# MAC-VO/MAC-VO

Measured on AMD Instinct MI355X. Metric: stereo frames/sec at 640x480 (hot path: cost volume + lookup, keypoint selection, covariance, PGO), higher is better.
Workload: dtype f32 via f16x2 (volume: fp32 operands row-scaled by powers of two and split into two fp16 pieces, three products, fp32 accumulate, scales undone exactly) + f32 (lookup/covariance) + f64 (PGO)

## Files before the change

mac-vo_amd/csrc/common.h:

```cpp
#pragma once
#include <hip/hip_runtime.h>
#include <stdint.h>
#include "macvo_hip.h"

#define MV_WAVE 64

#ifndef MV_PLAIN_STORES
#define MV_VOL_STORE(v, p) __builtin_nontemporal_store((v), (p))
#define MV_VOL_STORE_ASM_MOD " nt"
#else
#define MV_VOL_STORE(v, p) (*(p) = (v))
#define MV_VOL_STORE_ASM_MOD ""
#endif

struct mvEpiArgs {
    const float* flow;
    const float* logcov;
    int cov_is_log;
    float bl_fx, bl_fx_sq;
    float *disparity, *disparity_cov, *depth, *depth_cov, *match_flow, *match_cov;
    uint8_t* bad_mask;
};
#ifdef __HIPCC__
__device__ __forceinline__ void mv_epilogue_pixel(const mvEpiArgs& a, int plane, int i) {
    const float fx0 = a.flow[i];
    const float lc0 = a.logcov[i];
    const float dcov = a.cov_is_log ? expf(lc0 * 2.f) : lc0;
    const float d = fabsf(fx0);
    if (a.disparity) a.disparity[i] = d;
    if (a.disparity_cov) a.disparity_cov[i] = dcov;
    if (a.depth) a.depth[i] = a.bl_fx * (1.f / d);
    if (a.depth_cov) {
        const float d2 = d * d;
        const float err2 = dcov * (1.f / d2);
        a.depth_cov[i] = a.bl_fx_sq * (err2 / d2);
    }
    if (a.bad_mask) a.bad_mask[i] = fx0 <= 0.f;
    if (a.match_flow) {
        a.match_flow[i] = a.flow[2 * plane + i];
        a.match_flow[plane + i] = a.flow[3 * plane + i];
    }
    if (a.match_cov) {
        const float l0 = a.logcov[2 * plane + i], l1 = a.logcov[3 * plane + i];
        a.match_cov[i] = a.cov_is_log ? expf(l0 * 2.f) : l0;
        a.match_cov[plane + i] = a.cov_is_log ? expf(l1 * 2.f) : l1;
        a.match_cov[2 * plane + i] = 0.f;
    }
}
template <bool D, bool M>
__device__ __forceinline__ void mv_epilogue_pixel_partial(const mvEpiArgs& a, int plane, int i) {
    const float fx0 = a.flow[i];
    const float d = fabsf(fx0);
    if (a.disparity) a.disparity[i] = d;
    if (a.depth) a.depth[i] = a.bl_fx * (1.f / d);
    if constexpr (D) {
        const float lc0 = a.logcov[i];
        const float dcov = a.cov_is_log ? expf(lc0 * 2.f) : lc0;
        if (a.disparity_cov) a.disparity_cov[i] = dcov;
        if (a.depth_cov) {
            const float d2 = d * d;
            const float err2 = dcov * (1.f / d2);
            a.depth_cov[i] = a.bl_fx_sq * (err2 / d2);
        }
    }
    if (a.bad_mask) a.bad_mask[i] = fx0 <= 0.f;
    if (a.match_flow) {
        a.match_flow[i] = a.flow[2 * plane + i];
        a.match_flow[plane + i] = a.flow[3 * plane + i];
    }
    if constexpr (M) {
        if (a.match_cov) {
            const float l0 = a.logcov[2 * plane + i], l1 = a.logcov[3 * plane + i];
            a.match_cov[i] = a.cov_is_log ? expf(l0 * 2.f) : l0;
            a.match_cov[plane + i] = a.cov_is_log ? expf(l1 * 2.f) : l1;
            a.match_cov[2 * plane + i] = 0.f;
        }
    }
}
#endif

struct mvLaneCounts {
    int32_t n[MV_MAX_LANES];
};

#define MV_CHECK_ARG(cond) \
    do {                   \
        if (!(cond)) return MV_ERR_INVALID_ARG; \
    } while (0)

#ifndef MV_NO_SMALL_PRIO
#define MV_SMALL_KERNEL_PRIO() __builtin_amdgcn_s_setprio(3)
#else
#define MV_SMALL_KERNEL_PRIO() ((void)0)
#endif

#ifdef MV_PRIO_CHAIN
#define MV_CHAIN_KERNEL_PRIO() __builtin_amdgcn_s_setprio(3)
#else
#define MV_CHAIN_KERNEL_PRIO() ((void)0)
#endif

static inline int mv_launch_status() {
    return hipGetLastError() == hipSuccess ? MV_OK : MV_ERR_LAUNCH;
}

static inline int mv_ceil_div(int a, int b) { return (a + b - 1) / b; }

static inline bool mv_cov_modifiers_ok(int32_t m) {
    bool ended = false;
    for (int s = 0; s < 8; ++s) {
        const int k = (int)(((uint32_t)m >> (4 * s)) & 15u);
        if (k == 0) { ended = true; continue; }
        if (ended || s >= 4 || (k != MV_COVMOD_DIAG && k != MV_COVMOD_NORMALIZE)) return false;
    }
    return true;
}

#include "backend_desc.h"

__device__ __forceinline__ float wave_sum(float v) {
#pragma unroll
    for (int o = 32; o > 0; o >>= 1) v += __shfl_xor(v, o, 64);
    return v;
}
__device__ __forceinline__ double wave_sum(double v) {
#pragma unroll
// ... 9 lines not shown
```

mac-vo_amd/csrc/corr_lookup.hip:

```cpp
#include "common.h"

namespace {

struct AxisEntry { float w; int c; };

template <int K, int QPW, int STRIDE, int CELLS>
__device__ __forceinline__ void tap_pairs(const float* blk, const AxisEntry (*ax)[2 * K], int lane, float (&res)[(QPW * K * K + 63) / 64]) {
    constexpr int KK = K * K, NPAIR = QPW * KK, NR = (NPAIR + 63) / 64;
#pragma unroll
    for (int r = 0; r < NR; ++r) {
        const int pair = min(r * 64 + lane, NPAIR - 1);
        const int s = pair / KK, tap = pair - s * KK;
        const int ti = tap / K, tj = tap - ti * K;
        const AxisEntry X = ax[s][ti], Y = ax[s][K + tj];
        const float w = X.w, n = Y.w;
        const bool inblk = ((X.c & Y.c) & 256) != 0;
        const float* p = &blk[s * CELLS + (Y.c & 255) * STRIDE + (X.c & 255)];
        const float e = 1.f - w, so = 1.f - n;
        const float vnw = inblk ? p[0] : 0.f, vne = inblk ? p[1] : 0.f;
        const float vsw = inblk ? p[STRIDE] : 0.f, vse = inblk ? p[STRIDE + 1] : 0.f;
        float r0 = vnw * (so * e);
        r0 = r0 + vne * (so * w);
        r0 = r0 + vsw * (n * e);
        r0 = r0 + vse * (n * w);
        res[r] = r0;
    }
}

template <int K, int QPW, int QPB>
__device__ __forceinline__ void tap_pairs_out(float (*outs)[QPB + 1], int wave, int lane, const float (&res)[(QPW * K * K + 63) / 64]) {
    constexpr int KK = K * K, NPAIR = QPW * KK, NR = (NPAIR + 63) / 64;
#pragma unroll
    for (int r = 0; r < NR; ++r) {
        const int pair = r * 64 + lane;
        if (pair < NPAIR) {
            const int s = pair / KK, tap = pair - s * KK;
            outs[tap][wave * QPW + s] = res[r];
        }
    }
}

template <int R, int QPW, int QPB, typename VT = float>
__global__ __launch_bounds__(64 * (QPB / QPW)) void corr_lookup_kernel(const VT* __restrict__ vol,
                                                                        const float* __restrict__ coords,
                                                                        float* __restrict__ out, int N1, int H2, int W2) {
    constexpr int K = 2 * R + 1;
    constexpr int KK = K * K;
    constexpr int BS = K + 3;
    constexpr int CELLS = BS * BS;
    constexpr int NWAVE = QPB / QPW;
    constexpr int NTHR = 64 * NWAVE;
    constexpr int RPR = 64 / BS;
    constexpr int LPR = RPR * BS;
    constexpr int NROUND = (BS + RPR - 1) / RPR;
    constexpr bool TRIM = (BS - 2) % RPR == 0;
    constexpr int NINNER = (BS - 2) / RPR;
    constexpr int QPA = 64 / (2 * K);
    constexpr int APASS = (QPW + QPA - 1) / QPA;
    static_assert(QPW <= 32 && (QPW & (QPW - 1)) == 0 && QPB % QPW == 0, "bad lookup tiling");

    constexpr int BLK_STRIDE = QPW * CELLS;
    constexpr int BLK_FLOATS = NWAVE * BLK_STRIDE;
    constexpr int OUT_FLOATS = KK * (QPB + 1);
    __shared__ float smem[BLK_FLOATS > OUT_FLOATS ? BLK_FLOATS : OUT_FLOATS];
    float* blk = smem + (threadIdx.x >> 6) * BLK_STRIDE;
    float (*outs)[QPB + 1] = reinterpret_cast<float (*)[QPB + 1]>(smem);

    MV_SMALL_KERNEL_PRIO();
    const int b = blockIdx.y;
    const int q0 = blockIdx.x * QPB;
    const int t = threadIdx.x, lane = t & 63, wave = t >> 6;
    const int slice = H2 * W2;

    const int qmine = q0 + wave * QPW + (lane & (QPW - 1));
    float x = 0.f, y = 0.f;
    if (qmine < N1) {
        x = coords[((size_t)b * 2 + 0) * N1 + qmine];
        y = coords[((size_t)b * 2 + 1) * N1 + qmine];
    }
    const float xc = fminf(fmaxf(x, -1.0e6f), 1.0e6f), yc = fminf(fmaxf(y, -1.0e6f), 1.0e6f);
    const int bx = ((xc == xc) ? (int)floorf(xc) : 0) - R - 1;
    const int by = ((yc == yc) ? (int)floorf(yc) : 0) - R - 1;
    const float frx = xc - floorf(xc), fry = yc - floorf(yc);
    const int margin = ((frx < 0.01f) ? 1 : 0) | ((frx > 0.99f) ? 2 : 0) | ((fry < 0.01f) ? 4 : 0) | ((fry > 0.99f) ? 8 : 0);

    const int cyl = lane / BS, cxl = lane - cyl * BS;
    float v[QPW][NROUND];
#pragma unroll
    for (int s = 0; s < QPW; ++s) {
        const int sbx = __builtin_amdgcn_readlane(bx, s), sby = __builtin_amdgcn_readlane(by, s);
        const int q = q0 + wave * QPW + s;
        const VT* __restrict__ base = vol + ((size_t)b * N1 + q) * slice;
        const int gx = sbx + cxl;
        if (TRIM) {
            const int mg = __builtin_amdgcn_readlane(margin, s);
            const bool okx = lane < LPR && q < N1 && gx >= 0 && gx < W2 && (cxl != 0 || (mg & 1)) && (cxl != BS - 1 || (mg & 2));
#pragma unroll
            for (int k = 0; k < NINNER; ++k) {
                const int row = 1 + k * RPR + cyl, gy = sby + row;
                const bool ok = okx && gy >= 0 && gy < H2;
                v[s][k] = ok ? (float)base[gy * W2 + gx] : 0.f;
            }
            v[s][NROUND - 1] = 0.f;
            if (mg & 12) {
                const int row = cyl == 0 ? 0 : BS - 1, gy = sby + row;
                const bool ok = okx && cyl < 2 && ((mg >> (cyl == 0 ? 2 : 3)) & 1) && gy >= 0 && gy < H2;
                v[s][NROUND - 1] = ok ? (float)base[gy * W2 + gx] : 0.f;
            }
        } else {
            const bool okx = lane < LPR && q < N1 && gx >= 0 && gx < W2;
#pragma unroll
            for (int k = 0; k < NROUND; ++k) {
                const int row = k * RPR + cyl, gy = sby + row;
                const bool ok = okx && row < BS && gy >= 0 && gy < H2;
                v[s][k] = ok ? (float)base[gy * W2 + gx] : 0.f;
            }
        }
    }

    const float wm1 = (float)(W2 - 1), hm1 = (float)(H2 - 1);
    const int asq = lane / (2 * K), aa = lane - asq * (2 * K);
    const bool a_is_y = aa >= K;
    const int aoff = (a_is_y ? aa - K : aa) - R;
    const float adim = a_is_y ? hm1 : wm1;
    __shared__ AxisEntry ax_all[NWAVE][QPW][2 * K];
    AxisEntry (*ax)[2 * K] = ax_all[wave];
#pragma unroll
    for (int ps = 0; ps < APASS; ++ps) {
        const int s = ps * QPA + asq;
        const float qx = __shfl(x, s, 64), qy = __shfl(y, s, 64);
        const int obx = __shfl(bx, s, 64), oby = __shfl(by, s, 64);
        const float cs = (a_is_y ? qy : qx) + (float)aoff;
        const float g = (2.f * cs) / adim - 1.f;
        const float ic = (g + 1.f) * (adim / 2.f);
        const float f0 = floorf(ic);
        const int c = (int)fminf(fmaxf(f0, -2.0e6f), 2.0e6f) - (a_is_y ? oby : obx);
        const bool inb = c >= 0 && c <= BS - 2;
        if (asq < QPA && s < QPW) ax[s][aa] = AxisEntry{ic - f0, min(max(c, 0), BS - 2) | (inb ? 256 : 0)};
    }

#pragma unroll
    for (int s = 0; s < QPW; ++s) {
        if (TRIM) {
#pragma unroll
            for (int k = 0; k < NINNER; ++k)
                if (lane < LPR) blk[s * CELLS + BS + k * LPR + lane] = v[s][k];
            if (lane < 2 * BS) blk[s * CELLS + (lane < BS ? lane : (BS - 2) * BS + lane)] = v[s][NROUND - 1];
        } else {
#pragma unroll
            for (int k = 0; k < NROUND; ++k)
                if (lane < LPR && k * LPR + lane < CELLS) blk[s * CELLS + k * LPR + lane] = v[s][k];
        }
    }
    __syncthreads();

    float res[(QPW * KK + 63) / 64];
    tap_pairs<K, QPW, BS, CELLS>(blk, ax, lane, res);
    __syncthreads();
    tap_pairs_out<K, QPW, QPB>(outs, wave, lane, res);
    __syncthreads();

    for (int idx = t; idx < KK * QPB; idx += NTHR) {
        const int k = idx / QPB, c = idx - k * QPB;
        if (q0 + c < N1) out[((size_t)b * KK + k) * N1 + q0 + c] = outs[k][c];
    }
}


template <int QPW, int QPB, typename VT = float>
__global__ __launch_bounds__(64 * (QPB / QPW)) void corr_lookup_tiled_kernel(const VT* __restrict__ vol,
                                                                              const float* __restrict__ coords,
                                                                              float* __restrict__ out, int N1, int H2, int W2) {
    constexpr int R = 4, K = 9, KK = 81;
    constexpr int BS = 16;
    constexpr int BSP = 18, CELLS = BS * BSP;
    constexpr int NWAVE = QPB / QPW, NTHR = 64 * NWAVE;
    constexpr int QPA = 64 / (2 * K);
    constexpr int APASS = (QPW + QPA - 1) / QPA;
    constexpr int BLK_STRIDE = QPW * CELLS;
    constexpr int BLK_FLOATS = NWAVE * BLK_STRIDE;
    constexpr int OUT_FLOATS = KK * (QPB + 1);
    __shared__ float smem[BLK_FLOATS > OUT_FLOATS ? BLK_FLOATS : OUT_FLOATS];
    float* blk = smem + (threadIdx.x >> 6) * BLK_STRIDE;
    float (*outs)[QPB + 1] = reinterpret_cast<float (*)[QPB + 1]>(smem);

    MV_SMALL_KERNEL_PRIO();
    const int b = blockIdx.y;
    const int q0 = blockIdx.x * QPB;
    const int t = threadIdx.x, lane = t & 63, wave = t >> 6;
    const int tpr = W2 >> 2, tpc = (H2 + 3) >> 2, slice = tpc * tpr * 16;

    const int qmine = q0 + wave * QPW + (lane & (QPW - 1));
    float x = 0.f, y = 0.f;
    if (qmine < N1) {
        x = coords[((size_t)b * 2 + 0) * N1 + qmine];
        y = coords[((size_t)b * 2 + 1) * N1 + qmine];
    }
    const float xc = fminf(fmaxf(x, -1.0e6f), 1.0e6f), yc = fminf(fmaxf(y, -1.0e6f), 1.0e6f);
    const int bx = ((xc == xc) ? (int)floorf(xc) : 0) - R - 1;
    const int by = ((yc == yc) ? (int)floorf(yc) : 0) - R - 1;
    const float frx = xc - floorf(xc), fry = yc - floorf(yc);
    const int x_lo = bx + ((frx < 0.01f) ? 0 : 1), x_hi = bx + ((frx > 0.99f) ? K + 2 : K + 1);
    const int y_lo = by + ((fry < 0.01f) ? 0 : 1), y_hi = by + ((fry > 0.99f) ? K + 2 : K + 1);
    const int tox = bx >> 2, toy = by >> 2;

    constexpr bool H16 = sizeof(VT) == 2;
    constexpr int NLD = H16 ? 2 : 4;
    const int ti = H16 ? (lane >> 3) & 3 : lane >> 4, cell = H16 ? (lane & 7) * 2 : lane & 15;
    const int half_row = H16 ? lane >> 5 : 0;
    float v[QPW][4];
#pragma unroll
    for (int s = 0; s < QPW; ++s) {
        const int stx = __builtin_amdgcn_readlane(tox, s), sty = __builtin_amdgcn_readlane(toy, s);
        const int sxl = __builtin_amdgcn_readlane(x_lo, s), sxh = __builtin_amdgcn_readlane(x_hi, s);
        const int syl = __builtin_amdgcn_readlane(y_lo, s), syh = __builtin_amdgcn_readlane(y_hi, s);
        const int q = q0 + wave * QPW + s;
        const VT* __restrict__ base = vol + ((size_t)b * N1 + q) * slice;
        const int tx = stx + ti;
        const bool okx = q < N1 && tx >= 0 && tx < tpr && 4 * tx + 3 >= sxl && 4 * tx <= sxh;
#pragma unroll
        for (int k = 0; k < NLD; ++k) {
            const int ty = sty + (H16 ? 2 * k + half_row : k);
            const bool ok = okx && ty >= 0 && ty < tpc && 4 * ty + 3 >= syl && 4 * ty <= syh;
            if constexpr (H16) {
                union { uint32_t u; _Float16 h[2]; } two;
                two.u = ok ? *reinterpret_cast<const uint32_t*>(base + ((ty * tpr + tx) << 4) + cell) : 0u;
                v[s][2 * k] = (float)two.h[0];
                v[s][2 * k + 1] = (float)two.h[1];
            } else {
                v[s][k] = ok ? (float)base[((ty * tpr + tx) << 4) + cell] : 0.f;
            }
        }
    }

    const float wm1 = (float)(W2 - 1), hm1 = (float)(H2 - 1);
    const int asq = lane / (2 * K), aa = lane - asq * (2 * K);
    const bool a_is_y = aa >= K;
    const int aoff = (a_is_y ? aa - K : aa) - R;
    const float adim = a_is_y ? hm1 : wm1;
    __shared__ AxisEntry ax_all[NWAVE][QPW][2 * K];
    AxisEntry (*ax)[2 * K] = ax_all[wave];
#pragma unroll
    for (int ps = 0; ps < APASS; ++ps) {
        const int s = ps * QPA + asq;
        const float qx = __shfl(x, s, 64), qy = __shfl(y, s, 64);
        const int obx = __shfl(tox, s, 64) * 4, oby = __shfl(toy, s, 64) * 4;
        const float cs = (a_is_y ? qy : qx) + (float)aoff;
        const float g = (2.f * cs) / adim - 1.f;
        const float ic = (g + 1.f) * (adim / 2.f);
        const float f0 = floorf(ic);
        const int c = (int)fminf(fmaxf(f0, -2.0e6f), 2.0e6f) - (a_is_y ? oby : obx);
        const bool inb = c >= 0 && c <= BS - 2;
        if (asq < QPA && s < QPW) ax[s][aa] = AxisEntry{ic - f0, min(max(c, 0), BS - 2) | (inb ? 256 : 0)};
    }

#pragma unroll
    for (int s = 0; s < QPW; ++s)
#pragma unroll
        for (int k = 0; k < NLD; ++k) {
            if constexpr (H16)
                *reinterpret_cast<float2*>(&blk[s * CELLS + (4 * (2 * k + half_row) + (cell >> 2)) * BSP + 4 * ti + (cell & 3)]) =
                    make_float2(v[s][2 * k], v[s][2 * k + 1]);
            else
                blk[s * CELLS + (4 * k + (cell >> 2)) * BSP + 4 * ti + (cell & 3)] = v[s][k];
        }
    __syncthreads();

    float res[(QPW * KK + 63) / 64];
    tap_pairs<K, QPW, BSP, CELLS>(blk, ax, lane, res);
    __syncthreads();
    tap_pairs_out<K, QPW, QPB>(outs, wave, lane, res);
    __syncthreads();
    for (int idx = t; idx < KK * QPB; idx += NTHR) {
        const int k = idx / QPB, c = idx - k * QPB;
        if (q0 + c < N1) out[((size_t)b * KK + k) * N1 + q0 + c] = outs[k][c];
    }
}

}

#include <stdlib.h>
static int lookup_small_threshold() {
    static int v = -1;
    if (v < 0) {
        const char* e = getenv("MV_LOOKUP_SMALL");
        v = e ? atoi(e) : 65536;
    }
    return v;
}

extern "C" int mv_corr_lookup(const float* vol, const float* coords, float* out, int B, int H1, int W1,
                              int H2, int W2, int radius, mvStream_t stream) {
    MV_CHECK_ARG(vol && coords && out);
    MV_CHECK_ARG(B > 0 && H1 > 0 && W1 > 0 && H2 > 1 && W2 > 1);
    if (radius < 1 || radius > 4) return MV_ERR_UNSUPPORTED;
    if (B > 65535) return MV_ERR_UNSUPPORTED;
    const int N1 = H1 * W1;
    hipStream_t s = (hipStream_t)stream;
    const bool small = (size_t)B * N1 <= (size_t)lookup_small_threshold();
    static int small_qpb = -1;
    if (small_qpb < 0) { const char* e = getenv("MV_LOOKUP_QPB"); small_qpb = (e && atoi(e) == 8) ? 8 : 16; }
#define MV_LOOKUP(R)                                                                                                  \
    if (small && small_qpb == 8)                                                                                      \
        hipLaunchKernelGGL((corr_lookup_kernel<R, 2, 8>), dim3(mv_ceil_div(N1, 8), B), dim3(256), 0, s, vol, coords,  \
                           out, N1, H2, W2);                                                                          \
    else if (small)                                                                                                   \
        hipLaunchKernelGGL((corr_lookup_kernel<R, 2, 16>), dim3(mv_ceil_div(N1, 16), B), dim3(512), 0, s, vol, coords, \
                           out, N1, H2, W2);                                                                          \
    else                                                                                                              \
        hipLaunchKernelGGL((corr_lookup_kernel<R, 4, 32>), dim3(mv_ceil_div(N1, 32), B), dim3(512), 0, s, vol, coords, \
                           out, N1, H2, W2)
    switch (radius) {
        case 1: MV_LOOKUP(1); break;
        case 2: MV_LOOKUP(2); break;
        case 3: MV_LOOKUP(3); break;
        default: MV_LOOKUP(4); break;
    }
#undef MV_LOOKUP
    return mv_launch_status();
}

extern "C" int mv_corr_lookup_vol16(const void* vol, const float* coords, float* out, int B, int H1, int W1, int H2, int W2, int radius,
                                    mvStream_t stream) {
    MV_CHECK_ARG(vol && coords && out);
    MV_CHECK_ARG(B > 0 && H1 > 0 && W1 > 0 && H2 > 1 && W2 > 1);
    if (radius != 4 || B > 65535) return MV_ERR_UNSUPPORTED;
    const int N1 = H1 * W1;
    hipStream_t s = (hipStream_t)stream;
    const _Float16* v = reinterpret_cast<const _Float16*>(vol);
    if ((size_t)B * N1 <= (size_t)lookup_small_threshold())
        hipLaunchKernelGGL((corr_lookup_kernel<4, 2, 16, _Float16>), dim3(mv_ceil_div(N1, 16), B), dim3(512), 0, s, v, coords, out, N1, H2, W2);
    else
        hipLaunchKernelGGL((corr_lookup_kernel<4, 4, 32, _Float16>), dim3(mv_ceil_div(N1, 32), B), dim3(512), 0, s, v, coords, out, N1, H2, W2);
    return mv_launch_status();
}

extern "C" int mv_corr_lookup_tiled(const float* vol, const float* coords, float* out, int B, int H1, int W1, int H2, int W2,
                                    int radius, mvStream_t stream) {
    MV_CHECK_ARG(vol && coords && out);
    MV_CHECK_ARG(B > 0 && H1 > 0 && W1 > 0 && H2 > 1 && W2 > 1);
    if (radius != 4 || (H2 % 4) || (W2 % 4) || B > 65535) return MV_ERR_UNSUPPORTED;
    const int N1 = H1 * W1;
    hipStream_t s = (hipStream_t)stream;
    if ((size_t)B * N1 <= (size_t)lookup_small_threshold())
        hipLaunchKernelGGL((corr_lookup_tiled_kernel<2, 16>), dim3(mv_ceil_div(N1, 16), B), dim3(512), 0, s, vol, coords, out, N1, H2, W2);
    else
        hipLaunchKernelGGL((corr_lookup_tiled_kernel<4, 32>), dim3(mv_ceil_div(N1, 32), B), dim3(512), 0, s, vol, coords, out, N1, H2, W2);
    return mv_launch_status();
}


extern "C" int mv_corr_lookup_tiled_vol16(const void* vol, const float* coords, float* out, int B, int H1, int W1, int H2, int W2, int radius,
                                          mvStream_t stream) {
    MV_CHECK_ARG(vol && coords && out);
    MV_CHECK_ARG(B > 0 && H1 > 0 && W1 > 0 && H2 > 1 && W2 > 1);
    MV_CHECK_ARG(((uintptr_t)vol & 31) == 0);
    if (radius != 4 || (W2 % 4) || B > 65535) return MV_ERR_UNSUPPORTED;
    const int N1 = H1 * W1;
    hipStream_t s = (hipStream_t)stream;
// ... 38 lines not shown
```

mac-vo_amd/csrc/kp_select.hip:

```cpp
#include "common.h"
#include <math.h>

namespace {

#ifdef MV_KP_PROFILE
__device__ long long g_kp_stamps[16];
#define KP_STAMP(i) do { if (threadIdx.x == 0) g_kp_stamps[i] = wall_clock64(); } while (0)
#else
#define KP_STAMP(i)
#endif

constexpr int TILE_W = 64;
constexpr int TILE_H = 16;
constexpr int MAX_R = 7;
constexpr unsigned CAND_FLAG = 0x80000000u;

struct KpWs {
    unsigned long long* cand_bits;
    unsigned* rec_idx;
    float* rec_q;
    float* rec_d;
    int* counters;
    size_t lane_bytes;

    __device__ __forceinline__ KpWs lane(int l) const {
        const size_t o = (size_t)l * lane_bytes;
        return KpWs{(unsigned long long*)((char*)cand_bits + o), (unsigned*)((char*)rec_idx + o), (float*)((char*)rec_q + o),
                    (float*)((char*)rec_d + o), (int*)((char*)counters + o), lane_bytes};
    }
};

__device__ __forceinline__ float flow_quality(const float* __restrict__ fc, int plane, int idx) {
    const float c0 = fc[idx], c1 = fc[plane + idx], c2 = fc[2 * plane + idx];
    return (c0 + c1) - 2.f * c2;
}

__device__ __forceinline__ float nanmin(float a, float b) { return (a < b || a != a) ? a : b; }

template <bool FUSE>
__global__ __launch_bounds__(256) void kp_nms_kernel(const float* __restrict__ fc, const float* __restrict__ d0,
                                                      const float* __restrict__ d0c, const float* __restrict__ d1,
                                                      const float* __restrict__ d1c,
                                                      const uint8_t* __restrict__ mask_a,
                                                      const uint8_t* __restrict__ mask_b, mvKpSelectParams p,
                                                      KpWs ws_all, int words_per_row, mvEpiArgs ef) {
    MV_CHAIN_KERNEL_PRIO();
    const KpWs ws = ws_all.lane(blockIdx.z);
    {
        const size_t lp = (size_t)blockIdx.z * p.H * p.W;
        if (fc) fc += 3 * lp;
        if (d0) d0 += lp;
        if (d0c) d0c += lp;
        if (d1) d1 += lp;
        if (d1c) d1c += lp;
        if (mask_a) mask_a += lp;
        if (mask_b) mask_b += lp;
        if (FUSE) {
            ef.flow += 4 * lp; ef.logcov += 4 * lp;
            if (ef.disparity) ef.disparity += lp;
            if (ef.disparity_cov) ef.disparity_cov += lp;
            if (ef.depth) ef.depth += lp;
            if (ef.depth_cov) ef.depth_cov += lp;
            if (ef.bad_mask) ef.bad_mask += lp;
            if (ef.match_flow) ef.match_flow += 2 * lp;
            if (ef.match_cov) ef.match_cov += 3 * lp;
        }
    }
    __shared__ float tile[TILE_H + 2 * MAX_R][TILE_W + 2 * MAX_R + 1];
    __shared__ float hmin[TILE_H + 2 * MAX_R][TILE_W + 1];
    __shared__ int wg_count, wg_base;
    const int H = p.H, W = p.W, plane = H * W;
    const int r = p.kernel_size >> 1;
    const int x0 = blockIdx.x * TILE_W, y0 = blockIdx.y * TILE_H;
    const int tx = threadIdx.x, ty = threadIdx.y;
    const int tid = ty * 64 + tx;
    const bool mapping = p.mode == MV_KP_MAPPING;
    if (tid == 0) wg_count = 0;

    if (!mapping) {
        const int tw = TILE_W + 2 * r, th = TILE_H + 2 * r;
        constexpr int NST = ((TILE_W + 2 * MAX_R) * (TILE_H + 2 * MAX_R) + 255) / 256;
        float qv[NST];
#pragma unroll
        for (int i = 0; i < NST; ++i) {
            const int e = i * 256 + tid;
            const int ly = e / tw, lx = e - ly * tw;
            const int gx = x0 + lx - r, gy = y0 + ly - r;
            float q = INFINITY;
            if (e < tw * th && gx >= 0 && gx < W && gy >= 0 && gy < H) {
                const int idx = gy * W + gx;
                if (FUSE) {
                    const float l0 = ef.logcov[2 * plane + idx], l1 = ef.logcov[3 * plane + idx];
                    const float c0 = ef.cov_is_log ? expf(l0 * 2.f) : l0, c1 = ef.cov_is_log ? expf(l1 * 2.f) : l1;
                    q = (c0 + c1) - 2.f * 0.f;
                } else if (p.mode == MV_KP_NODEPTH) {
                    q = flow_quality(fc, plane, idx);
                } else {
                    q = d0c[idx] + d1c[idx];
                    if (fc) q = q * flow_quality(fc, plane, idx);
                }
            }
            qv[i] = q;
        }
#pragma unroll
        for (int i = 0; i < NST; ++i) {
            const int e = i * 256 + tid;
            const int ly = e / tw, lx = e - ly * tw;
            if (e < tw * th) tile[ly][lx] = qv[i];
        }
        __syncthreads();
        for (int e = tid; e < th * TILE_W; e += 256) {
            const int ly = e >> 6, lx = e & 63;
            float m = tile[ly][lx];
            for (int dx = 1; dx <= 2 * r; ++dx) m = nanmin(m, tile[ly][lx + dx]);
            hmin[ly][lx] = m;
        }
    }
    __syncthreads();

    bool nms_px[TILE_H / 4];
    bool cand_px[TILE_H / 4];
    float q_px[TILE_H / 4];
    int my_nms = 0;
#pragma unroll
    for (int it = 0; it < TILE_H / 4; ++it) {
        const int ly = ty * (TILE_H / 4) + it;
        const int gx = x0 + tx, gy = y0 + ly;
        const bool inimg = gx < W && gy < H;
        const int idx = gy * W + gx;
        bool nms = false, cand = false;
        float q = 0.f;
        if (FUSE && inimg) mv_epilogue_pixel(ef, plane, idx);
        if (inimg) {
            const bool border = p.mask_width > 0 && gx >= p.mask_width && gx < W - p.mask_width &&
                                gy >= p.mask_width && gy < H - p.mask_width;
            if (mapping) {
                cand = border && (d0[idx] < p.max_depth) && (d0c[idx] < p.max_depth_cov);
            } else {
                q = tile[ly + r][tx + r];
                float m = hmin[ly][tx];
                for (int dy = 1; dy <= 2 * r; ++dy) m = nanmin(m, hmin[ly + dy][tx]);
                nms = (q == m);
                cand = nms && border;
                if (cand && p.mode == MV_KP_FULL) cand = (d0[idx] < p.max_depth) && (d1[idx] < p.max_depth);
            }
            if (cand && mask_a) cand = mask_a[idx] != 0;
            if (cand && mask_b) cand = mask_b[idx] != 0;
        }
        const unsigned long long cand_word = __ballot(cand);
        if (tx == 0 && gy < H) ws.cand_bits[(size_t)gy * words_per_row + blockIdx.x] = cand_word;
        nms_px[it] = nms;
        cand_px[it] = cand;
        q_px[it] = q;
        my_nms += nms;
    }
    if (mapping) return;

    int my_off = 0;
    if (my_nms) my_off = atomicAdd(&wg_count, my_nms);
    __syncthreads();
#ifdef MV_KP_FAKE_ATOMIC
    if (tid == 0) wg_base = (blockIdx.y * gridDim.x + blockIdx.x) * 16;
#else
    if (tid == 0) wg_base = wg_count ? atomicAdd(&ws.counters[0], wg_count) : 0;
#endif
    __syncthreads();
    int pos = wg_base + my_off;
#pragma unroll
    for (int it = 0; it < TILE_H / 4; ++it) {
        if (nms_px[it]) {
            const int gx = x0 + tx, gy = y0 + ty * (TILE_H / 4) + it;
            const int idx = gy * W + gx;
            ws.rec_idx[pos] = (unsigned)(((gy * words_per_row + blockIdx.x) << 6) | tx) | (cand_px[it] ? CAND_FLAG : 0u);
            if (p.mode == MV_KP_NODEPTH) {
                ws.rec_q[pos] = q_px[it];
            } else {
                ws.rec_q[pos] = fc ? flow_quality(fc, plane, idx) : 0.f;
                ws.rec_d[pos] = d0c[idx];
            }
            ++pos;
        }
    }
}

__device__ __forceinline__ unsigned float_key(float f) {
    if (f != f) return 0xFFFFFFFFu;
    const unsigned u = __float_as_uint(f);
    return (u & 0x80000000u) ? ~u : (u | 0x80000000u);
}
__device__ __forceinline__ float key_float(unsigned k) {
    const unsigned u = (k & 0x80000000u) ? (k & 0x7FFFFFFFu) : ~k;
    return __uint_as_float(u);
}

#ifndef MV_KP_FINISH_THREADS
#define MV_KP_FINISH_THREADS 1024
#endif

constexpr int RANK_CAP = 256;
constexpr unsigned NAN_KEY = 0xFFFFFFFFu;

template <int NT>
__device__ __forceinline__ int block_exclusive_scan(int v, int* wave_tot , int& total) {
    constexpr int NW = NT / 64;
    const int tid = threadIdx.x;
    int incl = v;
#pragma unroll
    for (int o = 1; o < 64; o <<= 1) {
        const int t = __shfl_up(incl, o, 64);
        if ((tid & 63) >= o) incl += t;
    }
    __syncthreads();
    if ((tid & 63) == 63) wave_tot[tid >> 6] = incl;
    __syncthreads();
    int off = 0;
    total = 0;
#pragma unroll
    for (int w = 0; w < NW; ++w) {
        const int t = wave_tot[w];
        if (w < (tid >> 6)) off += t;
        total += t;
    }
    return off + incl - v;
}

template <int NT, bool CACHED, int RPT, typename F>
__device__ __forceinline__ void for_each_key(const float* __restrict__ vals, int n, const unsigned (&keys)[RPT], F&& f) {
    const int tid = threadIdx.x;
    if (CACHED) {
        const int nr = (n + NT - 1) / NT;
#pragma unroll
        for (int r = 0; r < RPT; ++r)
            if (r < nr && r * NT + tid < n) f(keys[r]);
    } else {
        for (int i = tid; i < n; i += NT) f(float_key(vals[i]));
    }
}

struct MedianLds {
    unsigned hist[2048];
    unsigned lst[RANK_CAP];
    unsigned red_lo[16], red_hi[16];
    int red_cnt[16];
    int wave_tot[16];
    int sh[4];
    unsigned res;
};

template <int NT, bool CACHED, int RPT>
__device__ float block_nanmedian(const float* __restrict__ vals, int n, const unsigned (&keys)[RPT], MedianLds& L) {
    constexpr int NW = NT / 64, BPT = 2048 / NT;
    const int tid = threadIdx.x;
    unsigned lo = NAN_KEY, hi = 0u;
    int cnt = 0;
    for_each_key<NT, CACHED, RPT>(vals, n, keys, [&](unsigned k) {
        if (k != NAN_KEY) {
            lo = min(lo, k);
            hi = max(hi, k);
            ++cnt;
        }
    });
#pragma unroll
    for (int o = 32; o > 0; o >>= 1) {
        lo = min(lo, (unsigned)__shfl_xor((int)lo, o, 64));
// ... 459 lines not shown
```

Measured before the change: 7092.

## Reuse staged LDS blocks for lookup outputs and restructure NMS record compaction

The correlation lookup kernel now writes tap results back into each wave's own staged block region, using only a wave-level LDS handover instead of two block-wide barriers and a separate output array. It redistributes taps across lanes with padded strides to cut LDS bank conflicts, and remaps output channels. The keypoint NMS kernel replaces the shared atomic counter with per-wave ballot counts and mbcnt-based positions. It also issues the fused epilogue loads early and overlaps the epilogue stores with the global atomic. This adds complex lane-mapping logic that is specialised for K=9, which raises the risk of indexing mistakes.

```diff
diff --git a/mac-vo_amd/csrc/common.h b/mac-vo_amd/csrc/common.h
--- a/mac-vo_amd/csrc/common.h
+++ b/mac-vo_amd/csrc/common.h
@@ -42,6 +42,35 @@
     }
     if (a.match_cov) {
         const float l0 = a.logcov[2 * plane + i], l1 = a.logcov[3 * plane + i];
+        a.match_cov[i] = a.cov_is_log ? expf(l0 * 2.f) : l0;
+        a.match_cov[plane + i] = a.cov_is_log ? expf(l1 * 2.f) : l1;
+        a.match_cov[2 * plane + i] = 0.f;
+    }
+}
+struct mvEpiPixel { float fx0, lc0, f2, f3, l0, l1; };
+__device__ __forceinline__ mvEpiPixel mv_epilogue_load(const mvEpiArgs& a, int plane, int i) {
+    return mvEpiPixel{a.flow[i], a.logcov[i], a.flow[2 * plane + i], a.flow[3 * plane + i], a.logcov[2 * plane + i], a.logcov[3 * plane + i]};
+}
+__device__ __forceinline__ void mv_epilogue_store(const mvEpiArgs& a, int plane, int i, const mvEpiPixel& v) {
+    const float fx0 = v.fx0;
+    const float lc0 = v.lc0;
+    const float dcov = a.cov_is_log ? expf(lc0 * 2.f) : lc0;
+    const float d = fabsf(fx0);
+    if (a.disparity) a.disparity[i] = d;
+    if (a.disparity_cov) a.disparity_cov[i] = dcov;
+    if (a.depth) a.depth[i] = a.bl_fx * (1.f / d);
+    if (a.depth_cov) {
+        const float d2 = d * d;
+        const float err2 = dcov * (1.f / d2);
+        a.depth_cov[i] = a.bl_fx_sq * (err2 / d2);
+    }
+    if (a.bad_mask) a.bad_mask[i] = fx0 <= 0.f;
+    if (a.match_flow) {
+        a.match_flow[i] = v.f2;
+        a.match_flow[plane + i] = v.f3;
+    }
+    if (a.match_cov) {
+        const float l0 = v.l0, l1 = v.l1;
         a.match_cov[i] = a.cov_is_log ? expf(l0 * 2.f) : l0;
         a.match_cov[plane + i] = a.cov_is_log ? expf(l1 * 2.f) : l1;
         a.match_cov[2 * plane + i] = 0.f;
diff --git a/mac-vo_amd/csrc/corr_lookup.hip b/mac-vo_amd/csrc/corr_lookup.hip
--- a/mac-vo_amd/csrc/corr_lookup.hip
+++ b/mac-vo_amd/csrc/corr_lookup.hip
@@ -2,41 +2,98 @@
 
 namespace {
 
-struct AxisEntry { float w; int c; };
+struct alignas(8) AxisEntry { float w; int c; };
+
+__device__ __forceinline__ void wave_lds_handover() {
+    __builtin_amdgcn_fence(__ATOMIC_RELEASE, "wavefront");
+    __builtin_amdgcn_wave_barrier();
+    __builtin_amdgcn_fence(__ATOMIC_ACQUIRE, "wavefront");
+}
+
+template <int K, int STRIDE>
+__device__ __forceinline__ float tap_one(const float* qblk, const AxisEntry* qax, int ti, int tj) {
+    const AxisEntry X = qax[ti], Y = qax[K + tj];
+    const float w = X.w, n = Y.w;
+    const bool inblk = ((X.c & Y.c) & 256) != 0;
+    const float* p = &qblk[(Y.c & 255) * STRIDE + (X.c & 255)];
+    const float e = 1.f - w, so = 1.f - n;
+    const float vnw = inblk ? p[0] : 0.f, vne = inblk ? p[1] : 0.f;
+    const float vsw = inblk ? p[STRIDE] : 0.f, vse = inblk ? p[STRIDE + 1] : 0.f;
+    float r0 = vnw * (so * e);
+    r0 = r0 + vne * (so * w);
+    r0 = r0 + vsw * (n * e);
+    r0 = r0 + vse * (n * w);
+    return r0;
+}
+
+template <int K, int QPW>
+constexpr int strip_pitch() { return K * K + ((K == 9 && QPW == 4) ? 2 : 1); }
+template <int K, int QPW, int CELLS>
+constexpr int wave_floats() { return QPW * CELLS + ((K == 9 && QPW == 4) ? 12 : 0); }
+
+template <int K>
+__device__ __forceinline__ int tap_channel(int u) {
+    if constexpr (K == 9) return u < 72 ? u + (u >> 3) : 9 * (u - 72) + 8;
+    else return u;
+}
 
 template <int K, int QPW, int STRIDE, int CELLS>
-__device__ __forceinline__ void tap_pairs(const float* blk, const AxisEntry (*ax)[2 * K], int lane, float (&res)[(QPW * K * K + 63) / 64]) {
-    constexpr int KK = K * K, NPAIR = QPW * KK, NR = (NPAIR + 63) / 64;
-#pragma unroll
-    for (int r = 0; r < NR; ++r) {
-        const int pair = min(r * 64 + lane, NPAIR - 1);
-        const int s = pair / KK, tap = pair - s * KK;
-        const int ti = tap / K, tj = tap - ti * K;
-        const AxisEntry X = ax[s][ti], Y = ax[s][K + tj];
-        const float w = X.w, n = Y.w;
-        const bool inblk = ((X.c & Y.c) & 256) != 0;
-        const float* p = &blk[s * CELLS + (Y.c & 255) * STRIDE + (X.c & 255)];
-        const float e = 1.f - w, so = 1.f - n;
-        const float vnw = inblk ? p[0] : 0.f, vne = inblk ? p[1] : 0.f;
-        const float vsw = inblk ? p[STRIDE] : 0.f, vse = inblk ? p[STRIDE + 1] : 0.f;
-        float r0 = vnw * (so * e);
-        r0 = r0 + vne * (so * w);
-        r0 = r0 + vsw * (n * e);
-        r0 = r0 + vse * (n * w);
-        res[r] = r0;
-    }
-}
-
-template <int K, int QPW, int QPB>
-__device__ __forceinline__ void tap_pairs_out(float (*outs)[QPB + 1], int wave, int lane, const float (&res)[(QPW * K * K + 63) / 64]) {
-    constexpr int KK = K * K, NPAIR = QPW * KK, NR = (NPAIR + 63) / 64;
-#pragma unroll
-    for (int r = 0; r < NR; ++r) {
-        const int pair = r * 64 + lane;
-        if (pair < NPAIR) {
-            const int s = pair / KK, tap = pair - s * KK;
-            outs[tap][wave * QPW + s] = res[r];
+__device__ __forceinline__ void tap_phase(float* blk, const AxisEntry (*ax)[2 * K], int lane) {
+    constexpr int KK = K * K, P = strip_pitch<K, QPW>();
+    static_assert(P <= CELLS, "the output strip must fit in the wave's staged blocks");
+    if constexpr (K == 9) {
+        static_assert(QPW % 2 == 0, "the leftover rounds pair queries");
+        constexpr int NL = QPW / 2;
+        float res[QPW + NL];
+        const int ti0 = lane >> 3, tj0 = lane & 7;
+#pragma unroll
+        for (int r = 0; r < QPW; ++r) res[r] = tap_one<K, STRIDE>(blk + r * CELLS, ax[r], ti0, tj0);
+        const int l = lane & 31;
+        const bool rowh = lane >= 32;
+        const int sl = rowh ? (l >= 9 ? 1 : 0) : ((l >> 3) & 1);
+        const int ti = rowh ? min(l - 9 * sl, 8) : 8, tj = rowh ? 8 : (l & 7);
+        const bool live = rowh ? l < 18 : l < 16;
+        const int ul = sl * P + (rowh ? 72 + ti : 64 + tj);
+#pragma unroll
+        for (int m = 0; m < NL; ++m) res[QPW + m] = tap_one<K, STRIDE>(blk + (2 * m + sl) * CELLS, ax[2 * m + sl], ti, tj);
+        wave_lds_handover();
+#pragma unroll
+        for (int r = 0; r < QPW; ++r) blk[r * P + lane] = res[r];
+#pragma unroll
+        for (int m = 0; m < NL; ++m)
+            if (live) blk[2 * m * P + ul] = res[QPW + m];
+    } else {
+        constexpr int NPAIR = QPW * KK, NR = (NPAIR + 63) / 64;
+        constexpr int D0 = 64 % K, D1 = (64 / K) % K, D2 = 64 / KK;
+        float res[NR];
+        int oaddr[NR];
+        int s = lane / KK, ti = (lane - s * KK) / K, tj = lane - s * KK - ti * K;
+#pragma unroll
+        for (int r = 0; r < NR; ++r) {
+            const int sc = min(s, QPW - 1);
+            res[r] = tap_one<K, STRIDE>(blk + sc * CELLS, ax[sc], ti, tj);
+            oaddr[r] = s < QPW ? s * P + ti * K + tj : -1;
+            tj += D0;
+            const int c0 = tj >= K ? 1 : 0;
+            tj -= c0 * K;
+            ti += D1 + c0;
+            const int c1 = ti >= K ? 1 : 0;
+            ti -= c1 * K;
+            s += D2 + c1;
         }
+        wave_lds_handover();
+#pragma unroll
+        for (int r = 0; r < NR; ++r)
+            if (oaddr[r] >= 0) blk[oaddr[r]] = res[r];
+    }
+}
+
+template <int K, int QPW, int QPB, int BLK_STRIDE>
+__device__ __forceinline__ void store_tokens(const float* smem, float* __restrict__ out, int b, int q0, int N1, int t) {
+    constexpr int KK = K * K, P = strip_pitch<K, QPW>(), NTHR = 64 * (QPB / QPW);
+    for (int idx = t; idx < KK * QPB; idx += NTHR) {
+        const int u = idx / QPB, c = idx - u * QPB;
+        if (q0 + c < N1) out[((size_t)b * KK + tap_channel<K>(u)) * N1 + q0 + c] = smem[(c / QPW) * BLK_STRIDE + (c % QPW) * P + u];
     }
 }
 
@@ -45,11 +102,9 @@
                                                                         const float* __restrict__ coords,
                                                                         float* __restrict__ out, int N1, int H2, int W2) {
     constexpr int K = 2 * R + 1;
-    constexpr int KK = K * K;
     constexpr int BS = K + 3;
-    constexpr int CELLS = BS * BS;
+    constexpr int CELLS = BS * BS + (K == 9 ? 2 : 0);
     constexpr int NWAVE = QPB / QPW;
-    constexpr int NTHR = 64 * NWAVE;
     constexpr int RPR = 64 / BS;
     constexpr int LPR = RPR * BS;
     constexpr int NROUND = (BS + RPR - 1) / RPR;
@@ -59,12 +114,9 @@
     constexpr int APASS = (QPW + QPA - 1) / QPA;
     static_assert(QPW <= 32 && (QPW & (QPW - 1)) == 0 && QPB % QPW == 0, "bad lookup tiling");
 
-    constexpr int BLK_STRIDE = QPW * CELLS;
-    constexpr int BLK_FLOATS = NWAVE * BLK_STRIDE;
-    constexpr int OUT_FLOATS = KK * (QPB + 1);
-    __shared__ float smem[BLK_FLOATS > OUT_FLOATS ? BLK_FLOATS : OUT_FLOATS];
+    constexpr int BLK_STRIDE = wave_floats<K, QPW, CELLS>();
+    __shared__ float smem[NWAVE * BLK_STRIDE];
     float* blk = smem + (threadIdx.x >> 6) * BLK_STRIDE;
-    float (*outs)[QPB + 1] = reinterpret_cast<float (*)[QPB + 1]>(smem);
 
     MV_SMALL_KERNEL_PRIO();
     const int b = blockIdx.y;
@@ -149,21 +201,15 @@
         } else {
 #pragma unroll
             for (int k = 0; k < NROUND; ++k)
-                if (lane < LPR && k * LPR + lane < CELLS) blk[s * CELLS + k * LPR + lane] = v[s][k];
+                if (lane < LPR && k * LPR + lane < BS * BS) blk[s * CELLS + k * LPR + lane] = v[s][k];
         }
     }
+    wave_lds_handover();
+
+    tap_phase<K, QPW, BS, CELLS>(blk, ax, lane);
     __syncthreads();
 
-    float res[(QPW * KK + 63) / 64];
-    tap_pairs<K, QPW, BS, CELLS>(blk, ax, lane, res);
-    __syncthreads();
-    tap_pairs_out<K, QPW, QPB>(outs, wave, lane, res);
-    __syncthreads();
-
-    for (int idx = t; idx < KK * QPB; idx += NTHR) {
-        const int k = idx / QPB, c = idx - k * QPB;
-        if (q0 + c < N1) out[((size_t)b * KK + k) * N1 + q0 + c] = outs[k][c];
-    }
+    store_tokens<K, QPW, QPB, BLK_STRIDE>(smem, out, b, q0, N1, t);
 }
 
 
@@ -171,18 +217,15 @@
 __global__ __launch_bounds__(64 * (QPB / QPW)) void corr_lookup_tiled_kernel(const VT* __restrict__ vol,
                                                                               const float* __restrict__ coords,
                                                                               float* __restrict__ out, int N1, int H2, int W2) {
-    constexpr int R = 4, K = 9, KK = 81;
+    constexpr int R = 4, K = 9;
     constexpr int BS = 16;
-    constexpr int BSP = 18, CELLS = BS * BSP;
-    constexpr int NWAVE = QPB / QPW, NTHR = 64 * NWAVE;
+    constexpr int BSP = 20, CELLS = BS * BSP + 18;
+    constexpr int NWAVE = QPB / QPW;
     constexpr int QPA = 64 / (2 * K);
     constexpr int APASS = (QPW + QPA - 1) / QPA;
-    constexpr int BLK_STRIDE = QPW * CELLS;
-    constexpr int BLK_FLOATS = NWAVE * BLK_STRIDE;
-    constexpr int OUT_FLOATS = KK * (QPB + 1);
-    __shared__ float smem[BLK_FLOATS > OUT_FLOATS ? BLK_FLOATS : OUT_FLOATS];
+    constexpr int BLK_STRIDE = wave_floats<K, QPW, CELLS>();
+    __shared__ __attribute__((aligned(16))) float smem[NWAVE * BLK_STRIDE];
     float* blk = smem + (threadIdx.x >> 6) * BLK_STRIDE;
-    float (*outs)[QPB + 1] = reinterpret_cast<float (*)[QPB + 1]>(smem);
 
     MV_SMALL_KERNEL_PRIO();
     const int b = blockIdx.y;
@@ -264,17 +307,11 @@
             else
                 blk[s * CELLS + (4 * k + (cell >> 2)) * BSP + 4 * ti + (cell & 3)] = v[s][k];
         }
+    wave_lds_handover();
+
+    tap_phase<K, QPW, BSP, CELLS>(blk, ax, lane);
     __syncthreads();
-
-    float res[(QPW * KK + 63) / 64];
-    tap_pairs<K, QPW, BSP, CELLS>(blk, ax, lane, res);
-    __syncthreads();
-    tap_pairs_out<K, QPW, QPB>(outs, wave, lane, res);
-    __syncthreads();
-    for (int idx = t; idx < KK * QPB; idx += NTHR) {
-        const int k = idx / QPB, c = idx - k * QPB;
-        if (q0 + c < N1) out[((size_t)b * KK + k) * N1 + q0 + c] = outs[k][c];
-    }
+    store_tokens<K, QPW, QPB, BLK_STRIDE>(smem, out, b, q0, N1, t);
 }
 
 }
diff --git a/mac-vo_amd/csrc/kp_select.hip b/mac-vo_amd/csrc/kp_select.hip
--- a/mac-vo_amd/csrc/kp_select.hip
+++ b/mac-vo_amd/csrc/kp_select.hip
@@ -68,14 +68,13 @@
     }
     __shared__ float tile[TILE_H + 2 * MAX_R][TILE_W + 2 * MAX_R + 1];
     __shared__ float hmin[TILE_H + 2 * MAX_R][TILE_W + 1];
-    __shared__ int wg_count, wg_base;
+    __shared__ int wave_cnt[4], wg_base;
     const int H = p.H, W = p.W, plane = H * W;
     const int r = p.kernel_size >> 1;
     const int x0 = blockIdx.x * TILE_W, y0 = blockIdx.y * TILE_H;
     const int tx = threadIdx.x, ty = threadIdx.y;
     const int tid = ty * 64 + tx;
     const bool mapping = p.mode == MV_KP_MAPPING;
-    if (tid == 0) wg_count = 0;
 
     if (!mapping) {
         const int tw = TILE_W + 2 * r, th = TILE_H + 2 * r;
@@ -118,30 +117,51 @@
     }
     __syncthreads();
 
-    bool nms_px[TILE_H / 4];
-    bool cand_px[TILE_H / 4];
-    float q_px[TILE_H / 4];
-    int my_nms = 0;
-#pragma unroll
-    for (int it = 0; it < TILE_H / 4; ++it) {
-        const int ly = ty * (TILE_H / 4) + it;
-        const int gx = x0 + tx, gy = y0 + ly;
+    constexpr int NPX = TILE_H / 4;
+    const int gx = x0 + tx;
+
+    bool nms_px[NPX];
+    float q_px[NPX];
+    unsigned long long nms_word[NPX];
+#pragma unroll
+    for (int it = 0; it < NPX; ++it) {
+        const int ly = ty * NPX + it;
+        bool nms = false;
+        float q = 0.f;
+        if (!mapping && gx < W && y0 + ly < H) {
+            q = tile[ly + r][tx + r];
+            float m = hmin[ly][tx];
+            for (int dy = 1; dy <= 2 * r; ++dy) m = nanmin(m, hmin[ly + dy][tx]);
+            nms = (q == m);
+        }
+        nms_px[it] = nms;
+        q_px[it] = q;
+        nms_word[it] = __ballot(nms);
+    }
+
+    mvEpiPixel epi[NPX] = {};
+    if (FUSE) {
+#pragma unroll
+        for (int it = 0; it < NPX; ++it) {
+            const int gy = y0 + ty * NPX + it;
+            if (gx < W && gy < H) epi[it] = mv_epilogue_load(ef, plane, gy * W + gx);
+        }
+    }
+
+    bool cand_px[NPX];
+    auto pixel_rest = [&](int it) {
+        const int gy = y0 + ty * NPX + it;
         const bool inimg = gx < W && gy < H;
         const int idx = gy * W + gx;
-        bool nms = false, cand = false;
-        float q = 0.f;
-        if (FUSE && inimg) mv_epilogue_pixel(ef, plane, idx);
+        bool cand = false;
+        if (FUSE && inimg) mv_epilogue_store(ef, plane, idx, epi[it]);
         if (inimg) {
             const bool border = p.mask_width > 0 && gx >= p.mask_width && gx < W - p.mask_width &&
                                 gy >= p.mask_width && gy < H - p.mask_width;
             if (mapping) {
                 cand = border && (d0[idx] < p.max_depth) && (d0c[idx] < p.max_depth_cov);
             } else {
-                q = tile[ly + r][tx + r];
-                float m = hmin[ly][tx];
-                for (int dy = 1; dy <= 2 * r; ++dy) m = nanmin(m, hmin[ly + dy][tx]);
-                nms = (q == m);
-                cand = nms && border;
+                cand = nms_px[it] && border;
                 if (cand && p.mode == MV_KP_FULL) cand = (d0[idx] < p.max_depth) && (d1[idx] < p.max_depth);
             }
             if (cand && mask_a) cand = mask_a[idx] != 0;
@@ -149,37 +169,52 @@
         }
         const unsigned long long cand_word = __ballot(cand);
         if (tx == 0 && gy < H) ws.cand_bits[(size_t)gy * words_per_row + blockIdx.x] = cand_word;
-        nms_px[it] = nms;
         cand_px[it] = cand;
-        q_px[it] = q;
-        my_nms += nms;
-    }
-    if (mapping) return;
-
-    int my_off = 0;
-    if (my_nms) my_off = atomicAdd(&wg_count, my_nms);
+    };
+    if (!FUSE) {
+#pragma unroll
+        for (int it = 0; it < NPX; ++it) pixel_rest(it);
+        if (mapping) return;
+    }
+
+    int wave_n = 0;
+#pragma unroll
+    for (int it = 0; it < NPX; ++it) wave_n += __popcll(nms_word[it]);
+    if (tx == 0) wave_cnt[ty] = wave_n;
     __syncthreads();
+    const int n0 = wave_cnt[0], n1 = wave_cnt[1], n2 = wave_cnt[2], n3 = wave_cnt[3];
+    const int wg_n = n0 + n1 + n2 + n3;
+    int base = 0;
 #ifdef MV_KP_FAKE_ATOMIC
-    if (tid == 0) wg_base = (blockIdx.y * gridDim.x + blockIdx.x) * 16;
+    if (tid == 0) base = (blockIdx.y * gridDim.x + blockIdx.x) * 16;
 #else
-    if (tid == 0) wg_base = wg_count ? atomicAdd(&ws.counters[0], wg_count) : 0;
+    int opaque_zero = 0;
+    asm volatile("" : "+v"(opaque_zero));
+    if (tid == 0 && wg_n) base = atomicAdd(ws.counters + opaque_zero, wg_n);
 #endif
+    if (FUSE) {
+#pragma unroll
+        for (int it = 0; it < NPX; ++it) pixel_rest(it);
+    }
+    if (tid == 0) wg_base = base;
     __syncthreads();
-    int pos = wg_base + my_off;
-#pragma unroll
-    for (int it = 0; it < TILE_H / 4; ++it) {
+    int pos = wg_base + (ty > 0 ? n0 : 0) + (ty > 1 ? n1 : 0) + (ty > 2 ? n2 : 0);
+#pragma unroll
+    for (int it = 0; it < NPX; ++it) {
         if (nms_px[it]) {
-            const int gx = x0 + tx, gy = y0 + ty * (TILE_H / 4) + it;
+            const int gy = y0 + ty * NPX + it;
             const int idx = gy * W + gx;
-            ws.rec_idx[pos] = (unsigned)(((gy * words_per_row + blockIdx.x) << 6) | tx) | (cand_px[it] ? CAND_FLAG : 0u);
+            const int at = pos + (int)__builtin_amdgcn_mbcnt_hi((unsigned)(nms_word[it] >> 32),
+                                                                __builtin_amdgcn_mbcnt_lo((unsigned)nms_word[it], 0u));
+            ws.rec_idx[at] = (unsigned)(((gy * words_per_row + blockIdx.x) << 6) | tx) | (cand_px[it] ? CAND_FLAG : 0u);
             if (p.mode == MV_KP_NODEPTH) {
-                ws.rec_q[pos] = q_px[it];
+                ws.rec_q[at] = q_px[it];
             } else {
-                ws.rec_q[pos] = fc ? flow_quality(fc, plane, idx) : 0.f;
-                ws.rec_d[pos] = d0c[idx];
-            }
-            ++pos;
-        }
+                ws.rec_q[at] = fc ? flow_quality(fc, plane, idx) : 0.f;
+                ws.rec_d[at] = d0c[idx];
+            }
+        }
+        pos += __popcll(nms_word[it]);
     }
 }
 
diff --git a/profiles/probes/lookup_lds_bank_model.py b/profiles/probes/lookup_lds_bank_model.py
--- /dev/null
+++ b/profiles/probes/lookup_lds_bank_model.py
@@ -0,0 +1,163 @@
+#!/usr/bin/env python
+import itertools
+import sys
+
+K, KK = 9, 81
+
+
+def pitch(qpw):
+    return 83 if qpw == 4 else 82
+
+
+def wave_pad(qpw):
+    return 12 if qpw == 4 else 0
+
+
+def group_cycles(accesses, nbanks, width=1):
+    per_bank = {}
+    for a in set(accesses):
+        for d in range(width):
+            per_bank.setdefault((a + d) % nbanks, set()).add(a + d)
+    worst = max((len(v) for v in per_bank.values()), default=1)
+    return 1, worst - 1
+
+
+def stream(lanes_addr, nbanks=32, width=1, group=32):
+    base = extra = 0
+    for g0 in range(0, 64, group):
+        acc = [a for a in lanes_addr[g0:g0 + group] if a is not None]
+        if not acc:
+            continue
+        b, e = group_cycles(acc, nbanks, width)
+        base, extra = base + b, extra + e
+    return base, extra
+
+
+def deal_old(qpw):
+    npair = qpw * KK
+    rounds = []
+    for r in range((npair + 63) // 64):
+        row = []
+        for lane in range(64):
+            pair = min(r * 64 + lane, npair - 1)
+            s, tap = divmod(pair, KK)
+            ti, tj = divmod(tap, K)
+            row.append((s, ti, tj, r * 64 + lane < npair))
+        rounds.append(row)
+    return rounds
+
+
+def deal_new(qpw):
+    rounds = [[(r, lane >> 3, lane & 7, True) for lane in range(64)] for r in range(qpw)]
+    for m in range(qpw // 2):
+        row = []
+        for lane in range(64):
+            l, rowh = lane & 31, lane >= 32
+            sl = (1 if l >= 9 else 0) if rowh else (l >> 3) & 1
+            ti = min(l - 9 * sl, 8) if rowh else 8
+            tj = 8 if rowh else l & 7
+            row.append((2 * m + sl, ti, tj, l < 18 if rowh else l < 16))
+        rounds.append(row)
+    return rounds
+
+
+def tap_reads(rounds, stride, cells, offs, ax_base=0):
+    cb = ce = ab = ae = 0
+    for row in rounds:
+        for dy, dx in ((0, 0), (0, 1), (1, 0), (1, 1)):
+            b, e = stream([s * cells + (tj + offs[s][1] + dy) * stride + ti + offs[s][0] + dx for s, ti, tj, _ in row])
+            cb, ce = cb + b, ce + e
+        for sel in (0, 1):
+            b, e = stream([ax_base + 2 * (s * 2 * K + (ti if sel == 0 else K + tj)) for s, ti, tj, _ in row], nbanks=64, width=2)
+            ab, ae = ab + b, ae + e
+    return cb, ce, ab, ae
+
+
+def staging_stores(kind, new, qpw):
+    b = e = 0
+    if kind == "row":
+        cells = 146 if new else 144
+        for s in range(qpw):
+            for k in range(2):
+                bb, ee = stream([s * cells + 12 + k * 60 + lane if lane < 60 else None for lane in range(64)])
+                b, e = b + bb, e + ee
+    else:
+        bsp, cells = (20, 338) if new else (18, 288)
+        for s in range(qpw):
+            for k in range(4):
+                bb, ee = stream([s * cells + (4 * k + ((lane & 15) >> 2)) * bsp + 4 * (lane >> 4) + (lane & 3) for lane in range(64)])
+                b, e = b + bb, e + ee
+    return b, e
+
+
+def result_stores(rounds, new, qpw, qpb, wave=0):
+    b = e = 0
+    for row in rounds:
+        if new:
+            addr = [s * pitch(qpw) + (8 * ti + tj if tj < 8 else 72 + ti) if live else None for s, ti, tj, live in row]
+        else:
+            addr = [(ti * K + tj) * (qpb + 1) + wave * qpw + s if live else None for s, ti, tj, live in row]
+        bb, ee = stream(addr)
+        b, e = b + bb, e + ee
+    return b, e
+
+
+def final_reads(new, qpw, qpb, blk_stride):
+    nthr = 64 * (qpb // qpw)
+    b = e = 0
+    for w0 in range(0, KK * qpb, 64):
+        addr = []
+        for idx in range(w0, w0 + 64):
+            if idx >= KK * qpb:
+                addr.append(None)
+                continue
+            u, c = divmod(idx, qpb)
+            addr.append((c // qpw) * blk_stride + (c % qpw) * pitch(qpw) + u if new else u * (qpb + 1) + c)
+        bb, ee = stream(addr)
+        b, e = b + bb, e + ee
+    return b, e, nthr
+
+
+def report(kind, qpw, qpb):
+    out = []
+    for new in (False, True):
+        rounds = deal_new(qpw) if new else deal_old(qpw)
+        if kind == "row":
+            stride, cells = 12, (146 if new else 144)
+            offsets = [[(1, 1)] * qpw]
+        else:
+            stride, cells = (20, 338) if new else (18, 288)
+            pair = list(itertools.product(range(1, 5), repeat=4))
+            offsets = [[(p[0], p[1]), (p[2], p[3])] * (qpw // 2) for p in pair]
+        acc = [0, 0, 0, 0]
+        for offs in offsets:
+            for i, v in enumerate(tap_reads(rounds, stride, cells, offs)):
+                acc[i] += v / len(offsets)
+        sb, se = staging_stores(kind, new, qpw)
+        rb, re_ = result_stores(rounds, new, qpw, qpb)
+        fb, fe, _ = final_reads(new, qpw, qpb, qpw * cells + (wave_pad(qpw) if new else 0))
+        nwave = qpb // qpw
+        fb, fe = fb / nwave, fe / nwave
+        tot_b = acc[0] + acc[2] + sb + rb + fb
+        tot_e = acc[1] + acc[3] + se + re_ + fe
+        out.append((new, acc, (sb, se), (rb, re_), (fb, fe), tot_e / (tot_b + tot_e)))
+    print(f"{kind}-major kernel, QPW = {qpw}, QPB = {qpb}   (LDS-array cycles per wave: base + extra from conflicts)")
+    for new, acc, st, rs, fr, share in out:
+        print(f"  {'new' if new else 'old'}: cell reads {acc[0]:.0f} + {acc[1]:.2f}   axis reads {acc[2]:.0f} + {acc[3]:.2f}   staging stores {st[0]} + {st[1]}   "
+              f"result stores {rs[0]} + {rs[1]}   final reads {fr[0]:.1f} + {fr[1]:.1f}   conflict share {100 * share:.1f} %")
+    return out
+
+
+def main() -> int:
+    res = [report("row", 2, 16), report("row", 4, 32), report("tiled", 2, 16), report("tiled", 4, 32)]
+    ok = True
+    for (old, new) in ((r[0], r[1]) for r in res[:2]):
+        ok &= new[1][1] == 0 and new[1][3] == 0 and new[3][1] == 0 and new[2][1] <= old[2][1] and new[4][1] <= old[4][1]
+    for (old, new) in ((r[0], r[1]) for r in res[2:]):
+        ok &= new[1][1] < old[1][1] and new[2][1] <= old[2][1]
+    print("claims hold" if ok else "CLAIMS VIOLATED")
+    return 0 if ok else 1
+
+
+if __name__ == "__main__":
+    sys.exit(main())
diff --git a/profiles/probes/lookup_nms_alone.py b/profiles/probes/lookup_nms_alone.py
--- /dev/null
+++ b/profiles/probes/lookup_nms_alone.py
@@ -0,0 +1,78 @@
+#!/usr/bin/env python
+import argparse
+import os
+import statistics
+import sys
+
+sys.path.insert(0, os.path.dirname(os.path.dirname(os.path.dirname(os.path.abspath(__file__)))))
+import torch
+
+from macvo_amd import _lib as L
+from macvo_amd import ops
+
+
+def period(fn, reps, rounds):
+    for _ in range(20):
+        fn()
+    torch.cuda.synchronize()
+    out = []
+    for _ in range(rounds):
+        e0, e1 = torch.cuda.Event(enable_timing=True), torch.cuda.Event(enable_timing=True)
+        e0.record()
+        for _ in range(reps):
+            fn()
+        e1.record()
+        torch.cuda.synchronize()
+        out.append(e0.elapsed_time(e1) * 1e3 / reps)
+    return statistics.median(out), min(out), max(out)
+
+
+def main():
+    ap = argparse.ArgumentParser()
+    ap.add_argument("--reps", type=int, default=400)
+    ap.add_argument("--rounds", type=int, default=5)
+    a = ap.parse_args()
+    dev = torch.device("cuda:0")
+    lib = L.load()
+    print("library:", os.environ.get("MACVO_HIP_LIB") or L.LIB_PATH)
+    g = torch.Generator().manual_seed(0)
+    h8, w8 = 60, 80
+    for B in (2, 64):
+        vol = torch.randn(B * h8 * w8, 1, h8, w8, device=dev)
+        ys, xs = torch.meshgrid(torch.arange(h8), torch.arange(w8), indexing="ij")
+        coords = (torch.stack([xs, ys]).float()[None] + (torch.rand(B, 2, h8, w8, generator=g) * 2 - 1) * 8).to(dev)
+        tok = torch.empty(B, 81, h8, w8, device=dev)
+        s = ops._stream()
+        args = (vol.data_ptr(), coords.data_ptr(), tok.data_ptr(), B, h8, w8, h8, w8, 4, s)
+        med, lo, hi = period(lambda: lib.mv_corr_lookup(*args), a.reps if B == 2 else a.reps // 8, a.rounds)
+        print(f"lookup r=4 fp32 cells  B={B:2d}  {med:7.2f} us  [{lo:.2f} .. {hi:.2f}]")
+        del vol, coords, tok
+    H, W = 480, 640
+    flow = (torch.randn(2, 2, H, W, generator=g) * 4).to(dev)
+    cov = (torch.randn(2, 2, H, W, generator=g) * 0.5).to(dev)
+    med, lo, hi = period(lambda: ops.frontend_epilogue_select(flow, cov, 0.25, 320.0, kernel_size=7, mask_width=32, max_match_cov=100.0),
+                         a.reps // 4, a.rounds)
+    print(f"epilogue + selector, fused entry point (allocations of the wrapper included)  {med:7.2f} us  [{lo:.2f} .. {hi:.2f}]")
+    import ctypes as C
+    mk = lambda c: torch.empty(1, c, H, W, device=dev)
+    o = [mk(1), mk(1), mk(1), mk(1), mk(2), mk(3)]
+    p = L.mvKpSelectParams(H, W, L.MV_KP_NODEPTH, 7, 32, 0.0, 0.0, 100.0)
+    nbytes = lib.mv_kp_select_workspace_bytes(H, W)
+    ws = torch.zeros((nbytes + 7) // 8, dtype=torch.int64, device=dev)
+    cand = torch.empty(H * W, dtype=torch.int32, device=dev)
+    count, stats = torch.empty(4, dtype=torch.int32, device=dev), torch.empty(4, device=dev)
+    s = ops._stream()
+    fargs = (flow.data_ptr(), cov.data_ptr(), 1, 80.0, 6400.0, o[0].data_ptr(), o[1].data_ptr(), o[2].data_ptr(), o[3].data_ptr(), None,
+             o[4].data_ptr(), o[5].data_ptr(), None, None, C.byref(p), ws.data_ptr(), ws.numel() * 8, cand.data_ptr(), count.data_ptr(),
+             stats.data_ptr(), 1, s)
+    med, lo, hi = period(lambda: lib.mv_frontend_epilogue_select_lanes(*fargs), a.reps, a.rounds)
+    print(f"mv_frontend_epilogue_select_lanes (kp_nms_kernel<true> + finishing workgroup)  {med:7.2f} us  [{lo:.2f} .. {hi:.2f}]")
+    uargs = (o[5].data_ptr(), None, None, None, None, None, None, C.byref(p), ws.data_ptr(), ws.numel() * 8, cand.data_ptr(), count.data_ptr(),
+             stats.data_ptr(), 1, s)
+    med, lo, hi = period(lambda: lib.mv_kp_select_lanes(*uargs), a.reps, a.rounds)
+    print(f"mv_kp_select_lanes        (kp_nms_kernel<false> + finishing workgroup)         {med:7.2f} us  [{lo:.2f} .. {hi:.2f}]")
+    print("records / candidates of the last call:", int(count[1]), int(count[0]))
+
+
+if __name__ == "__main__":
+    main()
```

Result: faster. 7254, median of 6 (+2.3%).
